# Yxxxb/LAVT-RS

Hardware: NVIDIA B200
Metric: LAVT-RS fwd clips/s (8x384^2) (higher is better)
Workload: dtype bf16

## Files before the change

### include/lavt_b200.h

```cpp
#ifndef LAVT_B200_H_
#define LAVT_B200_H_

#include <stdint.h>

#ifdef __cplusplus
extern "C" {
#endif

#define LAVT_ABI_VERSION 3

#define LAVT_ERR_SHAPE 1
#define LAVT_ERR_CUDA 2
#define LAVT_ERR_ARCH 3

enum { LAVT_ACT_NONE = 0, LAVT_ACT_GELU = 1, LAVT_ACT_RELU = 2, LAVT_ACT_TANH = 3, LAVT_ACT_SIGMOID = 4 };

typedef struct lavt_win_geom {
  int32_t B, D, H, W;
  int32_t wd, wh, ww;
  int32_t sd, sh, sw;
  int32_t nwd, nwh, nww;
  int32_t N;
  int32_t Wd, Wh, Ww;
} lavt_win_geom_t;
// ... 20 lines not shown
int lavt_abi_version(void);
int lavt_check_device(void);

int lavt_gemm_bf16(const void* A, int64_t lda, const void* Wt, int64_t ldw, int32_t M, int32_t N, int32_t K,
                   const lavt_epilogue_t* epi, void* stream);

int lavt_conv3x3_bf16(const void* x_nhwc, int64_t ldx, int32_t n_img, int32_t H, int32_t W, int32_t Cin,
                      const void* Wt, int32_t Cout, const lavt_epilogue_t* epi, void* stream);

int lavt_conv3d_bf16(const void* x_ndhwc, int64_t ldx, int32_t n_clip, int32_t D, int32_t H, int32_t W, int32_t Cin,
                     const void* Wt, int32_t Cout, const lavt_epilogue_t* epi, void* stream);


int lavt_layernorm_rows(const float* x, int64_t ldx, int64_t M, int32_t C, const float* gamma, const float* beta,
                        float eps, void* out_bf16, float* out_f32, void* stream);

int lavt_layernorm_window_gather(const float* x, int32_t C, const lavt_win_geom_t* geom, const float* gamma,
                                 const float* beta, float eps, void* out_bf16, void* stream);

int lavt_patch_merge_layernorm(const float* x, int32_t B, int32_t D, int32_t H, int32_t W, int32_t C,
                               const float* gamma, const float* beta, float eps, void* out_bf16, void* stream);

int lavt_patch_embed_im2col(const float* x, int64_t stride_b, int64_t stride_c, int64_t stride_t, int32_t B, int32_t T,
                            int32_t H, int32_t W, void* out_bf16, void* stream);

int lavt_window_attention(const void* qkv, const float* table_t, int32_t L, int32_t nH, const lavt_win_geom_t* geom,
                          void* out_bf16, void* stream);
int lavt_window_attention_lse(const void* qkv, const float* table_t, int32_t L, int32_t nH, const lavt_win_geom_t* geom, void* out_bf16,
                              float* lse, void* stream);
int lavt_window_attention_has_lse(const lavt_win_geom_t* geom, int32_t L, int32_t nH);
// ... 160 lines not shown
```

### lavt_rs_b200/_cabi.py

```python
from __future__ import annotations

import ctypes as C
import os
from typing import Optional

import torch

_PKG = os.path.dirname(os.path.abspath(__file__))
LIB_PATH = os.environ.get("LAVT_LIB_PATH") or os.path.join(_PKG, "_lib", "liblavt_b200.so")

ACT_NONE, ACT_GELU, ACT_RELU, ACT_TANH, ACT_SIGMOID = 0, 1, 2, 3, 4


class WinGeom(C.Structure):
    _fields_ = [(n, C.c_int32) for n in
                ("B", "D", "H", "W", "wd", "wh", "ww", "sd", "sh", "sw",
                 "nwd", "nwh", "nww", "N", "Wd", "Wh", "Ww")]

    def rows(self) -> int:
        return self.B * self.nwd * self.nwh * self.nww * self.N

    def tokens(self) -> int:
        return self.B * self.D * self.H * self.W

# ... 36 lines not shown


ABI_VERSION = 3

_i32, _i64, _f32, _vp = C.c_int32, C.c_int64, C.c_float, C.c_void_p
_EP = C.POINTER(Epilogue)
_WG = C.POINTER(WinGeom)

SIGNATURES = {
    "lavt_check_device": [],
    "lavt_gemm_bf16": [_vp, _i64, _vp, _i64, _i32, _i32, _i32, _EP, _vp],
    "lavt_gemm_bf16_smallm": [_vp, _i64, _vp, _i64, _i32, _i32, _i32, _EP, _vp, _i64, _vp],
    "lavt_conv3x3_bf16": [_vp, _i64, _i32, _i32, _i32, _i32, _vp, _i32, _EP, _vp],
    "lavt_conv3d_bf16": [_vp, _i64, _i32, _i32, _i32, _i32, _i32, _vp, _i32, _EP, _vp],
    "lavt_layernorm_rows": [_vp, _i64, _i64, _i32, _vp, _vp, _f32, _vp, _vp, _vp],
    "lavt_layernorm_window_gather": [_vp, _i32, _WG, _vp, _vp, _f32, _vp, _vp],
    "lavt_patch_merge_layernorm": [_vp, _i32, _i32, _i32, _i32, _i32, _vp, _vp, _f32, _vp, _vp],
    "lavt_patch_embed_im2col": [_vp, _i64, _i64, _i64, _i32, _i32, _i32, _i32, _vp, _vp],
    "lavt_window_attention": [_vp, _vp, _i32, _i32, _WG, _vp, _vp],
    "lavt_window_attention_lse": [_vp, _vp, _i32, _i32, _WG, _vp, _vp, _vp],
    "lavt_instnorm_stats": [_vp, _i32, _i64, _i32, _f32, _vp, _vp, _vp],
    "lavt_pwam_kv": [_vp, _vp, _vp, _vp, _vp, _vp, _vp, _vp, _i32, _i32, _i32, _i32, _vp],
    "lavt_lang_project": [_vp, _vp, _vp, _vp, _vp, _vp, _vp, _i32, _i32, _i32, _i32, _vp],
    "lavt_lang_project_bwd": [_vp, _vp, _vp, _vp, _vp, _vp, _vp, _vp, _vp, _vp, _vp, _vp, _i32, _i32, _i32, _i32, _vp],
    "lavt_pwam_attend": [_vp, _vp, _vp, _vp, _vp, _vp, _i32, _i64, _i32, _i32, _i32, _vp],
    "lavt_pwam_mul_norm": [_vp, _vp, _vp, _vp, _i32, _i64, _i32, _vp],
    "lavt_instnorm_sum2": [_vp, _vp, _vp, _vp, _vp, _i32, _i64, _i32, _vp],
    "lavt_bert_embed": [_vp, _vp, _vp, _vp, _vp, _i32, _i32, _i32, _i32, _vp],
    "lavt_bert_attention": [_vp, _vp, _vp, _i32, _i32, _i32, _i32, _vp],
    "lavt_rows_to_channels_first": [_vp, _vp, _i32, _i32, _i32, _vp],
# ... 44 lines not shown
    "lavt_efn_norm_upsample": [_vp, _vp, _vp, _vp, _i32, _i64, _i32, _i32, _i32, _vp],
    "lavt_bcam_softmax_rows": [_vp, _i64, _vp, _i64, _vp, _i64, _i64, _i32, _vp],
    "lavt_bcam_transpose_pad": [_vp, _i64, _vp, _i64, _i32, _i64, _i32, _vp],
    "lavt_gemm_f32_ref": [_vp, _i64, _vp, _i64, _i32, _i32, _i32, _EP, _vp],
    "lavt_window_attention_f32_ref": [_vp, _vp, _i32, _i32, _WG, _vp, _vp],
    "lavt_layernorm_window_gather_f32": [_vp, _i32, _WG, _vp, _vp, _f32, _vp, _vp],
    "lavt_rows_affine_act": [_vp, _i32, _i64, _vp, _i64, _vp, _i64, _vp, _vp, _i32, _vp, _vp, _i64, _i64, _i32, _vp],
    "lavt_avgpool2_nhwc": [_vp, _i64, _vp, _i64, _i32, _i32, _i32, _i32, _vp],
    "lavt_append_coords": [_vp, _i64, _vp, _i32, _i32, _i32, _i32, _vp],
    "lavt_rows_add_table": [_vp, _i32, _i64, _vp, _i64, _vp, _vp, _i64, _i64, _i32, _vp],
    "lavt_mha_small": [_vp, _i64, _vp, _i64, _vp, _i64, _vp, _vp, _i64, _i32, _i32, _i32, _i32, _vp],
    "lavt_gate_transpose": [_vp, _i64, _vp, _i64, _vp, _i32, _i32, _i32, _vp],
}
EXPORTS = ["lavt_last_error", "lavt_abi_version", "lavt_instnorm_workspace_floats", "lavt_set_attention_impl", "lavt_set_attention_bwd_impl",
           "lavt_gemm_splitk_workspace_floats", "lavt_conv3x3_wgrad_workspace_floats", "lavt_gacd_workspace_floats", "lavt_conv3d_wgrad_workspace_floats", "lavt_adamw_chunk_elems", "lavt_window_attention_has_lse",
           *SIGNATURES.keys()]


def _declare(l: C.CDLL) -> None:
    l.lavt_abi_version.restype = C.c_int
    l.lavt_instnorm_workspace_floats.argtypes = [_i32, _i64, _i32]
    l.lavt_instnorm_workspace_floats.restype = C.c_int64
    l.lavt_gemm_splitk_workspace_floats.argtypes = [_i32, _i32, _i32]
    l.lavt_gemm_splitk_workspace_floats.restype = C.c_int64
    l.lavt_window_attention_has_lse.argtypes = [_WG, _i32, _i32]
    l.lavt_window_attention_has_lse.restype = C.c_int
    l.lavt_conv3x3_wgrad_workspace_floats.argtypes = [_i32, _i32, _i32, _i32, _i32]
    l.lavt_conv3x3_wgrad_workspace_floats.restype = C.c_int64
    l.lavt_conv3d_wgrad_workspace_floats.argtypes = [_i32, _i32, _i32, _i32, _i32, _i32]
    l.lavt_conv3d_wgrad_workspace_floats.restype = C.c_int64
    l.lavt_gacd_workspace_floats.argtypes = [_i32, _i64, _i32]
    l.lavt_gacd_workspace_floats.restype = C.c_int64
    l.lavt_adamw_chunk_elems.argtypes = []
    l.lavt_adamw_chunk_elems.restype = C.c_int
    l.lavt_set_attention_impl.argtypes = [_i32]
    l.lavt_set_attention_impl.restype = C.c_int
    l.lavt_set_attention_bwd_impl.argtypes = [_i32]
    l.lavt_set_attention_bwd_impl.restype = C.c_int
    for name, argtypes in SIGNATURES.items():
        fn = getattr(l, name)
        fn.argtypes = argtypes
# ... 179 lines not shown
        raise LavtError(f"{name} must be contiguous")
    return t


def layernorm_rows(x: torch.Tensor, gamma, beta, *, out_bf16=None, out_f32=None, eps: float = 1e-5) -> None:
    _req(x, torch.float32, "x")
    M, Cn = x.shape
    for t, dt, nm in ((out_bf16, torch.bfloat16, "out_bf16"), (out_f32, torch.float32, "out_f32")):
        if t is not None:
            _c(t, dt, nm)
    check(lib().lavt_layernorm_rows(x.data_ptr(), x.stride(0), M, Cn, _c(gamma, torch.float32, "gamma").data_ptr(),
                                    _c(beta, torch.float32, "beta").data_ptr(), eps, ptr(out_bf16), ptr(out_f32),
                                    stream_ptr()), "lavt_layernorm_rows")


def layernorm_window_gather(x: torch.Tensor, geom: WinGeom, gamma, beta, out_bf16: torch.Tensor, eps: float = 1e-5) -> None:
    _c(x, torch.float32, "x")
    Cn = x.shape[-1]
    if x.numel() != geom.tokens() * Cn or out_bf16.numel() != geom.rows() * Cn:
        raise LavtError("window gather: tensor sizes do not match the geometry")
    check(lib().lavt_layernorm_window_gather(x.data_ptr(), Cn, C.byref(geom), _c(gamma, torch.float32, "gamma").data_ptr(),
                                             _c(beta, torch.float32, "beta").data_ptr(), eps,
                                             _c(out_bf16, torch.bfloat16, "out").data_ptr(), stream_ptr()),
          "lavt_layernorm_window_gather")


def patch_merge_layernorm(x: torch.Tensor, B, D, H, W, gamma, beta, out_bf16: torch.Tensor, eps: float = 1e-5) -> None:
    _c(x, torch.float32, "x")
    Cn = x.shape[-1]
    check(lib().lavt_patch_merge_layernorm(x.data_ptr(), B, D, H, W, Cn, _c(gamma, torch.float32, "gamma").data_ptr(),
# ... 699 lines not shown
```

### lavt_rs_b200/csrc/cabi.cu

```cuda
#include "../../include/lavt_b200.h"
#include "common.cuh"
#include "gemm_tc.cuh"
#include "kernels.cuh"

#include <cstring>

namespace lavt {
const char* last_error();
int gemm_dispatch(const void* A, long long lda, const void* Bw, long long ldb, const GemmParams& p,
                  cudaStream_t stream);

static_assert(sizeof(lavt_win_geom_t) == sizeof(WinGeom), "public/private window geometry mismatch");

static int fill_epilogue(GemmParams& p, const lavt_epilogue_t* e) {
  LAVT_REQUIRE(e != nullptr, "epilogue pointer is NULL");
  p.cscale = e->cscale;
  p.bias = e->bias;
  p.act = e->act;
  p.mul = static_cast<const __nv_bfloat16*>(e->mul);
  p.ldm = e->ldm;
  p.mul_act = e->mul_act;
  p.out_pre = static_cast<__nv_bfloat16*>(e->out_pre);
  p.pre_mode = e->pre_mode;
  LAVT_REQUIRE(e->pre_mode == 0 || (e->pre_mode == 1 && e->out_pre && e->act == LAVT_ACT_GELU),
// ... 95 lines not shown
}

static inline cudaStream_t S(void* s) { return static_cast<cudaStream_t>(s); }
static inline const __nv_bfloat16* CB(const void* p) { return static_cast<const __nv_bfloat16*>(p); }
static inline __nv_bfloat16* MB(void* p) { return static_cast<__nv_bfloat16*>(p); }

int lavt_layernorm_rows(const float* x, int64_t ldx, int64_t M, int32_t C, const float* gamma, const float* beta,
                        float eps, void* out_bf16, float* out_f32, void* stream) {
  LnParams p;
  std::memset(&p, 0, sizeof(p));
  p.x = x; p.ldx = ldx; p.gamma = gamma; p.beta = beta; p.out_bf16 = MB(out_bf16); p.out_f32 = out_f32;
  p.M = M; p.C = C; p.eps = eps;
  return ln_rows_dispatch(MODE_IDENTITY, p, S(stream));
}

int lavt_layernorm_window_gather(const float* x, int32_t C, const lavt_win_geom_t* geom, const float* gamma,
                                 const float* beta, float eps, void* out_bf16, void* stream) {
  LAVT_REQUIRE(geom != nullptr, "window gather: geometry is NULL");
  LnParams p;
  std::memset(&p, 0, sizeof(p));
  std::memcpy(&p.win, geom, sizeof(WinGeom));
  p.x = x; p.ldx = C; p.gamma = gamma; p.beta = beta; p.out_bf16 = MB(out_bf16);
  p.M = 1LL * geom->B * geom->nwd * geom->nwh * geom->nww * geom->N; p.C = C; p.eps = eps;
  return ln_rows_dispatch(MODE_WINDOW, p, S(stream));
}

int lavt_patch_merge_layernorm(const float* x, int32_t B, int32_t D, int32_t H, int32_t W, int32_t C,
                               const float* gamma, const float* beta, float eps, void* out_bf16, void* stream) {
  LnParams p;
  std::memset(&p, 0, sizeof(p));
// ... 424 lines not shown
```

### lavt_rs_b200/csrc/common.cuh

```cuda
#pragma once

#include <cuda.h>
#include <cuda_bf16.h>
#include <cuda_runtime.h>
#include <stdint.h>
#include <string.h>

#define LAVT_OK 0
#define LAVT_ERR_SHAPE 1
#define LAVT_ERR_CUDA 2
#define LAVT_ERR_ARCH 3

namespace lavt {

void set_last_error(const char* fmt, ...);
int check_cuda(cudaError_t e, const char* what);
#define LAVT_CUDA(call)                                   \
  do {                                                    \
    int _rc = ::lavt::check_cuda((call), #call);          \
    if (_rc != LAVT_OK) return _rc;                       \
  } while (0)
#define LAVT_LAUNCH_CHECK(name)                           \
  do {                                                    \
    int _rc = ::lavt::check_cuda(cudaGetLastError(), name); \
// ... 75 lines not shown
}

__device__ __forceinline__ uint32_t pack_bf16x2(float lo, float hi) {
  __nv_bfloat162 v = __floats2bfloat162_rn(lo, hi);
  return *reinterpret_cast<uint32_t*>(&v);
}
__device__ __forceinline__ float2 unpack_bf16x2(uint32_t u) {
  __nv_bfloat162 v = *reinterpret_cast<__nv_bfloat162*>(&u);
  return __bfloat1622float2(v);
}

__device__ __forceinline__ float gelu_erf(float x) {
  return 0.5f * x * (1.0f + erff(x * 0.70710678118654752440f));
}

__device__ __forceinline__ void mbar_init(uint64_t* bar, uint32_t count) {
  asm volatile("mbarrier.init.shared::cta.b64 [%0], %1;" ::"r"(smem_u32(bar)), "r"(count));
}
__device__ __forceinline__ void fence_mbar_init() {
  asm volatile("fence.mbarrier_init.release.cluster;" ::: "memory");
}
__device__ __forceinline__ void mbar_expect_tx(uint64_t* bar, uint32_t bytes) {
  asm volatile("mbarrier.arrive.expect_tx.shared::cta.b64 _, [%0], %1;" ::"r"(smem_u32(bar)),
               "r"(bytes)
               : "memory");
}
__device__ __forceinline__ void mbar_arrive(uint64_t* bar) {
  asm volatile("mbarrier.arrive.shared::cta.b64 _, [%0];" ::"r"(smem_u32(bar)) : "memory");
}
__device__ __forceinline__ bool mbar_try_wait(uint64_t* bar, uint32_t parity) {
// ... 250 lines not shown
```

### lavt_rs_b200/csrc/gemm_tc.cu

```cuda
#include "common.cuh"
#include "gemm_tc.cuh"

#include <cstdio>
#include <cstdlib>
#include <cstring>

namespace lavt {

constexpr int GEMM_BM = 128;
constexpr int GEMM_BK = 64;

template <int GEMM_BN, int GEMM_STAGES, int EPI_WGS, int CTA2 = 0>
struct GemmSmem {
  static constexpr int A_BYTES = GEMM_BM * GEMM_BK * 2;
  static constexpr int B_BYTES = (CTA2 ? GEMM_BN / 2 : GEMM_BN) * GEMM_BK * 2;
  static constexpr int STAGE_BYTES = A_BYTES + B_BYTES;
  static constexpr int RING_BYTES = GEMM_STAGES * STAGE_BYTES;
  static constexpr int BAR_OFF = RING_BYTES;
  static constexpr int VEC_OFF = BAR_OFF + 256;
  static constexpr int VEC_TILE_BYTES = EPI_WGS * 2 * GEMM_BN * 4;
  static constexpr int TOTAL = VEC_OFF + VEC_TILE_BYTES + 1024 ;
  static constexpr int THREADS = 128 + 128 * EPI_WGS;
  static constexpr int MIN_CTAS = (EPI_WGS == 1) ? 2 : 1;
  static constexpr int ACC = (MIN_CTAS == 2) ? 2 : 512 / GEMM_BN;
};

__device__ __forceinline__ float ex2_approx(float x) {
  float y;
  asm("ex2.approx.ftz.f32 %0, %1;" : "=f"(y) : "f"(x));
  return y;
}
__device__ __forceinline__ float rcp_approx(float x) {
  float y;
  asm("rcp.approx.ftz.f32 %0, %1;" : "=f"(y) : "f"(x));
  return y;
}
__device__ __forceinline__ uint64_t pk2(float lo, float hi) {
  uint64_t r;
  asm("mov.b64 %0, {%1, %2};" : "=l"(r) : "f"(lo), "f"(hi));
  return r;
}
__device__ __forceinline__ void upk2(uint64_t v, float& lo, float& hi) { asm("mov.b64 {%0, %1}, %2;" : "=f"(lo), "=f"(hi) : "l"(v)); }
__device__ __forceinline__ uint64_t fma2(uint64_t a, uint64_t b, uint64_t c) {
  uint64_t r;
  asm("fma.rn.f32x2 %0, %1, %2, %3;" : "=l"(r) : "l"(a), "l"(b), "l"(c));
  return r;
}
__device__ __forceinline__ uint64_t mul2(uint64_t a, uint64_t b) {
  uint64_t r;
  asm("mul.rn.f32x2 %0, %1, %2;" : "=l"(r) : "l"(a), "l"(b));
  return r;
}
__device__ __forceinline__ void gelu_erf2(float& x0, float& x1) {
  const uint64_t x = pk2(x0, x1);
  float z0, z1;
  upk2(mul2(x, pk2(0.70710678118654752f, 0.70710678118654752f)), z0, z1);
  z0 = fminf(fmaxf(z0, -3.0f), 3.0f);
  z1 = fminf(fmaxf(z1, -3.0f), 3.0f);
  const uint64_t z = pk2(z0, z1);
  const uint64_t t = mul2(z, z);
  constexpr float K = 1.0000220904f;
  uint64_t p = pk2(4.0742095563e-08f * K, 4.0742095563e-08f * K);
  p = fma2(p, t, pk2(-1.9448222676e-06f * K, -1.9448222676e-06f * K));
  p = fma2(p, t, pk2(4.1060515983e-05f * K, 4.1060515983e-05f * K));
  p = fma2(p, t, pk2(-5.1103678896e-04f * K, -5.1103678896e-04f * K));
  p = fma2(p, t, pk2(4.2354270142e-03f * K, 4.2354270142e-03f * K));
  p = fma2(p, t, pk2(-2.5102860078e-02f * K, -2.5102860078e-02f * K));
  p = fma2(p, t, pk2(1.1107933337e-01f * K, 1.1107933337e-01f * K));
  p = fma2(p, t, pk2(-3.7531487405e-01f * K, -3.7531487405e-01f * K));
  p = fma2(p, t, pk2(1.1282684285e+00f * K, 1.1282684285e+00f * K));
  const uint64_t e = mul2(z, p);
  const uint64_t hx = mul2(x, pk2(0.5f, 0.5f));
  upk2(fma2(hx, e, hx), x0, x1);
}
__device__ __forceinline__ void gelu_both2(float& x0, float& x1, float& d0, float& d1) {
  const uint64_t x = pk2(x0, x1);
  float z0, z1;
  upk2(mul2(x, pk2(0.70710678118654752f, 0.70710678118654752f)), z0, z1);
  const uint64_t zz = pk2(z0, z1);
  float q0, q1;
  upk2(mul2(zz, zz), q0, q1);
  const float e0 = ex2_approx(-1.4426950408889634f * q0), e1 = ex2_approx(-1.4426950408889634f * q1);
  z0 = fminf(fmaxf(z0, -3.0f), 3.0f);
  z1 = fminf(fmaxf(z1, -3.0f), 3.0f);
  const uint64_t z = pk2(z0, z1);
  const uint64_t t = mul2(z, z);
  constexpr float K = 1.0000220904f;
  uint64_t p = pk2(4.0742095563e-08f * K, 4.0742095563e-08f * K);
// ... 4 lines not shown
  p = fma2(p, t, pk2(-2.5102860078e-02f * K, -2.5102860078e-02f * K));
  p = fma2(p, t, pk2(1.1107933337e-01f * K, 1.1107933337e-01f * K));
  p = fma2(p, t, pk2(-3.7531487405e-01f * K, -3.7531487405e-01f * K));
  p = fma2(p, t, pk2(1.1282684285e+00f * K, 1.1282684285e+00f * K));
  const uint64_t Phi = fma2(mul2(z, p), pk2(0.5f, 0.5f), pk2(0.5f, 0.5f));
  const uint64_t xs = mul2(x, pk2(0.3989422804014327f, 0.3989422804014327f));
  upk2(fma2(xs, pk2(e0, e1), Phi), d0, d1);
  upk2(mul2(x, Phi), x0, x1);
}
__device__ __forceinline__ void gelu_grad2(float& x0, float& x1) {
  float d0, d1;
  gelu_both2(x0, x1, d0, d1);
  x0 = d0;
  x1 = d1;
}
__device__ __forceinline__ void ldg_v8(uint32_t* r, const void* p) {
  asm volatile("ld.global.v8.b32 {%0, %1, %2, %3, %4, %5, %6, %7}, [%8];"
               : "=r"(r[0]), "=r"(r[1]), "=r"(r[2]), "=r"(r[3]), "=r"(r[4]), "=r"(r[5]), "=r"(r[6]), "=r"(r[7])
               : "l"(p));
}
__device__ __forceinline__ void stg_v8(void* p, const uint32_t* r) {
  asm volatile("st.global.v8.b32 [%0], {%1, %2, %3, %4, %5, %6, %7, %8};" ::"l"(p), "r"(r[0]), "r"(r[1]), "r"(r[2]),
               "r"(r[3]), "r"(r[4]), "r"(r[5]), "r"(r[6]), "r"(r[7])
               : "memory");
}
__device__ __forceinline__ float tanh_fast(float x) {
  const float e = ex2_approx(x * 2.8853900817779268f);
  return fmaf(-2.0f, rcp_approx(e + 1.0f), 1.0f);
}

template <int GEMM_BN, int GEMM_STAGES, int EPI_WGS, int CTA2 = 0, int SIMPLE = 0>
__global__ void __launch_bounds__(GemmSmem<GEMM_BN, GEMM_STAGES, EPI_WGS, CTA2>::THREADS, GemmSmem<GEMM_BN, GEMM_STAGES, EPI_WGS, CTA2>::MIN_CTAS)
gemm_bf16_tc_kernel(const __grid_constant__ CUtensorMap tmA, const __grid_constant__ CUtensorMap tmB,
                    const GemmParams p, const int m_tiles, const int vec_all, long long* const trace_buf) {
  using L = GemmSmem<GEMM_BN, GEMM_STAGES, EPI_WGS, CTA2>;
  const int crank = CTA2 ? static_cast<int>(cluster_ctarank()) : 0;
  const int wid0 = CTA2 ? static_cast<int>(blockIdx.x >> 1) : static_cast<int>(blockIdx.x);
  const int wstep = CTA2 ? static_cast<int>(gridDim.x >> 1) : static_cast<int>(gridDim.x);
  extern __shared__ uint8_t smem_raw[];
  uint8_t* smem = smem_raw + ((1024u - (smem_u32(smem_raw) & 1023u)) & 1023u);
// ... 576 lines not shown
```

### lavt_rs_b200/csrc/kernels.cuh

```cuda
#pragma once
#include "common.cuh"
#include "geom.cuh"

namespace lavt {

enum { MODE_IDENTITY = 0, MODE_WINDOW = 1, MODE_MERGE = 2 };

struct LnParams {
  const float* x;
  long long ldx;
  const float* gamma;
  const float* beta;
  __nv_bfloat16* out_bf16;
  float* out_f32;
  long long M;
  int C;
  float eps;
  WinGeom win;
  int mB, mD, mH, mW;
};
int ln_rows_dispatch(int mode, const LnParams& p, cudaStream_t st);
int im2col_patch4_dispatch(const float* x, long long sB, long long sC, long long sT, __nv_bfloat16* out, int B, int T, int H,
                           int W, cudaStream_t st);
long long colstats_workspace_floats(int B, long long n, int C);
int colstats_dispatch(const float* x, float* stats, float* workspace, int B, long long n, int C, float eps, cudaStream_t st);
int instnorm_sum2_dispatch(const float* a, const float* sa, const float* b, const float* sb, float* out, int B, long long n,
                           int C, cudaStream_t st);
int pwam_mul_dispatch(const __nv_bfloat16* vis, const float* lang, const float* stats, __nv_bfloat16* out, int B,
                      long long n, int C, cudaStream_t st);

struct AttnParams {
  const __nv_bfloat16* qkv;
  const float* table_t;
  __nv_bfloat16* out;
  int C, nH, L;
  WinGeom win;
  float* lse;
};
int window_attn_dispatch(const AttnParams& p, cudaStream_t st);
int attn_impl_setting(int set);
enum class AttnKernel { TC3, TC2, MMA };
AttnKernel window_attn_choose(const AttnParams& p);
bool window_attn_tc2_supported(const AttnParams& p);
int window_attn_tc2_dispatch(const AttnParams& p, cudaStream_t st);
// ... 104 lines not shown
```

### lavt_rs_b200/engine.py

```python
from __future__ import annotations

from typing import Dict, Optional, Sequence, Tuple

import torch

from . import _cabi as K
from .geometry import window_geometry

LAUNCHES = 0
PRECISION = "bf16"


def set_precision(mode: str) -> str:
    global PRECISION
    if mode not in ("bf16", "fp32"):
        raise ValueError("precision must be 'bf16' or 'fp32'")
    prev, PRECISION = PRECISION, mode
    return prev


def _count(n: int = 1) -> None:
    global LAUNCHES
    LAUNCHES += n

# ... 81 lines not shown
        return s, b
    qkv_s, qkv_b = pw.get("qkv_sb", [blk.attn.qkv.weight] + ([blk.attn.qkv.bias] if blk.attn.qkv.bias is not None else []), _qscale)
    proj_w = pw.get("proj_w", [blk.attn.proj.weight], lambda: _bf16(blk.attn.proj.weight))
    fc1_w = pw.get("fc1_w", [blk.mlp.fc1.weight], lambda: _bf16(blk.mlp.fc1.weight))
    fc2_w = pw.get("fc2_w", [blk.mlp.fc2.weight], lambda: _bf16(blk.mlp.fc2.weight))
    table_t = pw.get("table_t", [blk.attn.relative_position_bias_table],
                     lambda: _f32(blk.attn.relative_position_bias_table.t()))

    xw = ws.get("xw", (rows, C), torch.bfloat16, dev)
    K.layernorm_window_gather(x, geom, blk.norm1.weight, blk.norm1.bias, xw, eps=blk.norm1.eps)
    qkv = ws.get("qkv", (rows, 3 * C), torch.bfloat16, dev)
    K.gemm_bf16(xw, qkv_w, cscale=qkv_s, bias=qkv_b, out_bf16=qkv)
    att = ws.get("att", (rows, C), torch.bfloat16, dev)
    K.window_attention(qkv, table_t, geom, att)
    K.gemm_bf16(att, proj_w, bias=blk.attn.proj.bias.detach(), resid=x, out_f32=x, win=geom)
    h1 = ws.get("ln2", (n, C), torch.bfloat16, dev)
    K.layernorm_rows(x, blk.norm2.weight, blk.norm2.bias, out_bf16=h1, eps=blk.norm2.eps)
    hid = ws.get("hid", (n, fc1_w.shape[0]), torch.bfloat16, dev)
    K.gemm_bf16(h1, fc1_w, bias=blk.mlp.fc1.bias.detach(), act=K.ACT_GELU, out_bf16=hid)
    K.gemm_bf16(hid, fc2_w, bias=blk.mlp.fc2.bias.detach(), resid=x, out_f32=x, out_bf16=xb_out)
    _count(7)


def _swin_block_fp32(x: torch.Tensor, blk, geom, ws: Workspace, xb_out: Optional[torch.Tensor]) -> None:
    n, C = x.shape
    dev = x.device
    rows, nH = geom.rows(), blk.num_heads
    hd = C // nH
    s = torch.ones(3 * C, device=dev, dtype=torch.float32)
    s[:C] = hd ** -0.5 * 1.4426950408889634
# ... 684 lines not shown
```

Before: 281.7.

## Fuse Swin MLP (LayerNorm, fc1+GELU, fc2+residual) into one persistent tcgen05 kernel

Adds a persistent warp-specialized kernel that runs LayerNorm2, fc1 with GELU, and fc2 with bias and residual for Swin blocks with C in {128,256}. The hidden activation stays in tensor memory and shared memory instead of making a round trip through global memory. The kernel uses a TMA weight ring, double-buffered A tiles and TMEM accumulators, and the engine calls it in place of three launches. It adds a complex mbarrier pipeline, which brings deadlock risk, and it only covers the two smaller channel widths.

After: 287.2, median of 6. +1.9%, better.

```diff
diff --git a/include/lavt_b200.h b/include/lavt_b200.h
--- a/include/lavt_b200.h
+++ b/include/lavt_b200.h
@@ -58,6 +58,10 @@
 
 int lavt_layernorm_rows(const float* x, int64_t ldx, int64_t M, int32_t C, const float* gamma, const float* beta,
                         float eps, void* out_bf16, float* out_f32, void* stream);
+
+int lavt_swin_mlp_supported(int32_t C, int32_t hidden);
+int lavt_swin_mlp_bf16(float* x, int64_t M, int32_t C, int32_t hidden, const float* gamma, const float* beta, float eps, const void* w1,
+                       const float* b1, const void* w2, const float* b2, void* xb_out, void* stream);
 
 int lavt_layernorm_window_gather(const float* x, int32_t C, const lavt_win_geom_t* geom, const float* gamma,
                                  const float* beta, float eps, void* out_bf16, void* stream);
diff --git a/lavt_rs_b200/_cabi.py b/lavt_rs_b200/_cabi.py
--- a/lavt_rs_b200/_cabi.py
+++ b/lavt_rs_b200/_cabi.py
@@ -74,6 +74,7 @@
     "lavt_conv3x3_bf16": [_vp, _i64, _i32, _i32, _i32, _i32, _vp, _i32, _EP, _vp],
     "lavt_conv3d_bf16": [_vp, _i64, _i32, _i32, _i32, _i32, _i32, _vp, _i32, _EP, _vp],
     "lavt_layernorm_rows": [_vp, _i64, _i64, _i32, _vp, _vp, _f32, _vp, _vp, _vp],
+    "lavt_swin_mlp_bf16": [_vp, _i64, _i32, _i32, _vp, _vp, _f32, _vp, _vp, _vp, _vp, _vp, _vp],
     "lavt_layernorm_window_gather": [_vp, _i32, _WG, _vp, _vp, _f32, _vp, _vp],
     "lavt_patch_merge_layernorm": [_vp, _i32, _i32, _i32, _i32, _i32, _vp, _vp, _f32, _vp, _vp],
     "lavt_patch_embed_im2col": [_vp, _i64, _i64, _i64, _i32, _i32, _i32, _i32, _vp, _vp],
@@ -148,7 +149,7 @@
 }
 EXPORTS = ["lavt_last_error", "lavt_abi_version", "lavt_instnorm_workspace_floats", "lavt_set_attention_impl", "lavt_set_attention_bwd_impl",
            "lavt_gemm_splitk_workspace_floats", "lavt_conv3x3_wgrad_workspace_floats", "lavt_gacd_workspace_floats", "lavt_conv3d_wgrad_workspace_floats", "lavt_adamw_chunk_elems", "lavt_window_attention_has_lse",
-           *SIGNATURES.keys()]
+           "lavt_swin_mlp_supported", *SIGNATURES.keys()]
 
 
 def _declare(l: C.CDLL) -> None:
@@ -159,6 +160,8 @@
     l.lavt_gemm_splitk_workspace_floats.restype = C.c_int64
     l.lavt_window_attention_has_lse.argtypes = [_WG, _i32, _i32]
     l.lavt_window_attention_has_lse.restype = C.c_int
+    l.lavt_swin_mlp_supported.argtypes = [_i32, _i32]
+    l.lavt_swin_mlp_supported.restype = C.c_int
     l.lavt_conv3x3_wgrad_workspace_floats.argtypes = [_i32, _i32, _i32, _i32, _i32]
     l.lavt_conv3x3_wgrad_workspace_floats.restype = C.c_int64
     l.lavt_conv3d_wgrad_workspace_floats.argtypes = [_i32, _i32, _i32, _i32, _i32, _i32]
@@ -368,6 +371,30 @@
                                     stream_ptr()), "lavt_layernorm_rows")
 
 
+def swin_mlp_supported(C: int, hidden: int) -> bool:
+    return bool(lib().lavt_swin_mlp_supported(int(C), int(hidden)))
+
+
+def swin_mlp(x: torch.Tensor, gamma, beta, w1: torch.Tensor, b1, w2: torch.Tensor, b2, *, xb_out=None, eps: float = 1e-5) -> None:
+    _c(x, torch.float32, "x")
+    M, Cn = x.shape
+    _c(w1, torch.bfloat16, "w1")
+    _c(w2, torch.bfloat16, "w2")
+    hidden = w1.shape[0]
+    if tuple(w1.shape) != (hidden, Cn) or tuple(w2.shape) != (Cn, hidden):
+        raise LavtError(f"swin mlp: weight shapes {tuple(w1.shape)} / {tuple(w2.shape)} do not match C={Cn}")
+    if xb_out is not None and tuple(xb_out.shape) != (M, Cn):
+        raise LavtError("swin mlp: xb_out must have the shape of x")
+    t0 = TIMER.begin()
+    check(lib().lavt_swin_mlp_bf16(x.data_ptr(), M, Cn, hidden, _c(gamma, torch.float32, "gamma").data_ptr(),
+                                   _c(beta, torch.float32, "beta").data_ptr(), eps, w1.data_ptr(), _c(b1, torch.float32, "b1").data_ptr(),
+                                   w2.data_ptr(), _c(b2, torch.float32, "b2").data_ptr(),
+                                   ptr(_c(xb_out, torch.bfloat16, "xb_out") if xb_out is not None else None), stream_ptr()),
+          "lavt_swin_mlp_bf16")
+    TIMER.end(t0, "swin_mlp_tc_kernel", 4.0 * M * Cn * hidden, 8.0 * M * Cn + 4.0 * Cn * hidden + (2.0 * M * Cn if xb_out is not None else 0.0),
+              f"M{M} C{Cn} hidden{hidden}")
+
+
 def layernorm_window_gather(x: torch.Tensor, geom: WinGeom, gamma, beta, out_bf16: torch.Tensor, eps: float = 1e-5) -> None:
     _c(x, torch.float32, "x")
     Cn = x.shape[-1]
diff --git a/lavt_rs_b200/csrc/cabi.cu b/lavt_rs_b200/csrc/cabi.cu
--- a/lavt_rs_b200/csrc/cabi.cu
+++ b/lavt_rs_b200/csrc/cabi.cu
@@ -133,6 +133,18 @@
   return ln_rows_dispatch(MODE_IDENTITY, p, S(stream));
 }
 
+int lavt_swin_mlp_supported(int32_t C, int32_t hidden) { return swin_mlp_supported(C, hidden) ? 1 : 0; }
+
+int lavt_swin_mlp_bf16(float* x, int64_t M, int32_t C, int32_t hidden, const float* gamma, const float* beta, float eps, const void* w1,
+                       const float* b1, const void* w2, const float* b2, void* xb_out, void* stream) {
+  SwinMlpParams p;
+  std::memset(&p, 0, sizeof(p));
+  p.x = x; p.xb_out = MB(xb_out); p.gamma = gamma; p.beta = beta; p.eps = eps;
+  p.w1 = CB(w1); p.b1 = b1; p.w2 = CB(w2); p.b2 = b2;
+  p.M = M; p.C = C; p.hidden = hidden;
+  return swin_mlp_dispatch(p, S(stream));
+}
+
 int lavt_layernorm_window_gather(const float* x, int32_t C, const lavt_win_geom_t* geom, const float* gamma,
                                  const float* beta, float eps, void* out_bf16, void* stream) {
   LAVT_REQUIRE(geom != nullptr, "window gather: geometry is NULL");
diff --git a/lavt_rs_b200/csrc/common.cuh b/lavt_rs_b200/csrc/common.cuh
--- a/lavt_rs_b200/csrc/common.cuh
+++ b/lavt_rs_b200/csrc/common.cuh
@@ -113,6 +113,55 @@
   return 0.5f * x * (1.0f + erff(x * 0.70710678118654752440f));
 }
 
+__device__ __forceinline__ uint64_t pk2(float lo, float hi) {
+  uint64_t r;
+  asm("mov.b64 %0, {%1, %2};" : "=l"(r) : "f"(lo), "f"(hi));
+  return r;
+}
+__device__ __forceinline__ void upk2(uint64_t v, float& lo, float& hi) { asm("mov.b64 {%0, %1}, %2;" : "=f"(lo), "=f"(hi) : "l"(v)); }
+__device__ __forceinline__ uint64_t fma2(uint64_t a, uint64_t b, uint64_t c) {
+  uint64_t r;
+  asm("fma.rn.f32x2 %0, %1, %2, %3;" : "=l"(r) : "l"(a), "l"(b), "l"(c));
+  return r;
+}
+__device__ __forceinline__ uint64_t mul2(uint64_t a, uint64_t b) {
+  uint64_t r;
+  asm("mul.rn.f32x2 %0, %1, %2;" : "=l"(r) : "l"(a), "l"(b));
+  return r;
+}
+__device__ __forceinline__ void gelu_erf2(float& x0, float& x1) {
+  const uint64_t x = pk2(x0, x1);
+  float z0, z1;
+  upk2(mul2(x, pk2(0.70710678118654752f, 0.70710678118654752f)), z0, z1);
+  z0 = fminf(fmaxf(z0, -3.0f), 3.0f);
+  z1 = fminf(fmaxf(z1, -3.0f), 3.0f);
+  const uint64_t z = pk2(z0, z1);
+  const uint64_t t = mul2(z, z);
+  constexpr float K = 1.0000220904f;
+  uint64_t p = pk2(4.0742095563e-08f * K, 4.0742095563e-08f * K);
+  p = fma2(p, t, pk2(-1.9448222676e-06f * K, -1.9448222676e-06f * K));
+  p = fma2(p, t, pk2(4.1060515983e-05f * K, 4.1060515983e-05f * K));
+  p = fma2(p, t, pk2(-5.1103678896e-04f * K, -5.1103678896e-04f * K));
+  p = fma2(p, t, pk2(4.2354270142e-03f * K, 4.2354270142e-03f * K));
+  p = fma2(p, t, pk2(-2.5102860078e-02f * K, -2.5102860078e-02f * K));
+  p = fma2(p, t, pk2(1.1107933337e-01f * K, 1.1107933337e-01f * K));
+  p = fma2(p, t, pk2(-3.7531487405e-01f * K, -3.7531487405e-01f * K));
+  p = fma2(p, t, pk2(1.1282684285e+00f * K, 1.1282684285e+00f * K));
+  const uint64_t e = mul2(z, p);
+  const uint64_t hx = mul2(x, pk2(0.5f, 0.5f));
+  upk2(fma2(hx, e, hx), x0, x1);
+}
+__device__ __forceinline__ void ldg_v8(uint32_t* r, const void* p) {
+  asm volatile("ld.global.v8.b32 {%0, %1, %2, %3, %4, %5, %6, %7}, [%8];"
+               : "=r"(r[0]), "=r"(r[1]), "=r"(r[2]), "=r"(r[3]), "=r"(r[4]), "=r"(r[5]), "=r"(r[6]), "=r"(r[7])
+               : "l"(p));
+}
+__device__ __forceinline__ void stg_v8(void* p, const uint32_t* r) {
+  asm volatile("st.global.v8.b32 [%0], {%1, %2, %3, %4, %5, %6, %7, %8};" ::"l"(p), "r"(r[0]), "r"(r[1]), "r"(r[2]),
+               "r"(r[3]), "r"(r[4]), "r"(r[5]), "r"(r[6]), "r"(r[7])
+               : "memory");
+}
+
 __device__ __forceinline__ void mbar_init(uint64_t* bar, uint32_t count) {
   asm volatile("mbarrier.init.shared::cta.b64 [%0], %1;" ::"r"(smem_u32(bar)), "r"(count));
 }
diff --git a/lavt_rs_b200/csrc/gemm_tc.cu b/lavt_rs_b200/csrc/gemm_tc.cu
--- a/lavt_rs_b200/csrc/gemm_tc.cu
+++ b/lavt_rs_b200/csrc/gemm_tc.cu
@@ -34,44 +34,6 @@
   float y;
   asm("rcp.approx.ftz.f32 %0, %1;" : "=f"(y) : "f"(x));
   return y;
-}
-__device__ __forceinline__ uint64_t pk2(float lo, float hi) {
-  uint64_t r;
-  asm("mov.b64 %0, {%1, %2};" : "=l"(r) : "f"(lo), "f"(hi));
-  return r;
-}
-__device__ __forceinline__ void upk2(uint64_t v, float& lo, float& hi) { asm("mov.b64 {%0, %1}, %2;" : "=f"(lo), "=f"(hi) : "l"(v)); }
-__device__ __forceinline__ uint64_t fma2(uint64_t a, uint64_t b, uint64_t c) {
-  uint64_t r;
-  asm("fma.rn.f32x2 %0, %1, %2, %3;" : "=l"(r) : "l"(a), "l"(b), "l"(c));
-  return r;
-}
-__device__ __forceinline__ uint64_t mul2(uint64_t a, uint64_t b) {
-  uint64_t r;
-  asm("mul.rn.f32x2 %0, %1, %2;" : "=l"(r) : "l"(a), "l"(b));
-  return r;
-}
-__device__ __forceinline__ void gelu_erf2(float& x0, float& x1) {
-  const uint64_t x = pk2(x0, x1);
-  float z0, z1;
-  upk2(mul2(x, pk2(0.70710678118654752f, 0.70710678118654752f)), z0, z1);
-  z0 = fminf(fmaxf(z0, -3.0f), 3.0f);
-  z1 = fminf(fmaxf(z1, -3.0f), 3.0f);
-  const uint64_t z = pk2(z0, z1);
-  const uint64_t t = mul2(z, z);
-  constexpr float K = 1.0000220904f;
-  uint64_t p = pk2(4.0742095563e-08f * K, 4.0742095563e-08f * K);
-  p = fma2(p, t, pk2(-1.9448222676e-06f * K, -1.9448222676e-06f * K));
-  p = fma2(p, t, pk2(4.1060515983e-05f * K, 4.1060515983e-05f * K));
-  p = fma2(p, t, pk2(-5.1103678896e-04f * K, -5.1103678896e-04f * K));
-  p = fma2(p, t, pk2(4.2354270142e-03f * K, 4.2354270142e-03f * K));
-  p = fma2(p, t, pk2(-2.5102860078e-02f * K, -2.5102860078e-02f * K));
-  p = fma2(p, t, pk2(1.1107933337e-01f * K, 1.1107933337e-01f * K));
-  p = fma2(p, t, pk2(-3.7531487405e-01f * K, -3.7531487405e-01f * K));
-  p = fma2(p, t, pk2(1.1282684285e+00f * K, 1.1282684285e+00f * K));
-  const uint64_t e = mul2(z, p);
-  const uint64_t hx = mul2(x, pk2(0.5f, 0.5f));
-  upk2(fma2(hx, e, hx), x0, x1);
 }
 __device__ __forceinline__ void gelu_both2(float& x0, float& x1, float& d0, float& d1) {
   const uint64_t x = pk2(x0, x1);
@@ -106,16 +68,6 @@
   x0 = d0;
   x1 = d1;
 }
-__device__ __forceinline__ void ldg_v8(uint32_t* r, const void* p) {
-  asm volatile("ld.global.v8.b32 {%0, %1, %2, %3, %4, %5, %6, %7}, [%8];"
-               : "=r"(r[0]), "=r"(r[1]), "=r"(r[2]), "=r"(r[3]), "=r"(r[4]), "=r"(r[5]), "=r"(r[6]), "=r"(r[7])
-               : "l"(p));
-}
-__device__ __forceinline__ void stg_v8(void* p, const uint32_t* r) {
-  asm volatile("st.global.v8.b32 [%0], {%1, %2, %3, %4, %5, %6, %7, %8};" ::"l"(p), "r"(r[0]), "r"(r[1]), "r"(r[2]),
-               "r"(r[3]), "r"(r[4]), "r"(r[5]), "r"(r[6]), "r"(r[7])
-               : "memory");
-}
 __device__ __forceinline__ float tanh_fast(float x) {
   const float e = ex2_approx(x * 2.8853900817779268f);
   return fmaf(-2.0f, rcp_approx(e + 1.0f), 1.0f);
diff --git a/lavt_rs_b200/csrc/kernels.cuh b/lavt_rs_b200/csrc/kernels.cuh
--- a/lavt_rs_b200/csrc/kernels.cuh
+++ b/lavt_rs_b200/csrc/kernels.cuh
@@ -28,6 +28,22 @@
                            int C, cudaStream_t st);
 int pwam_mul_dispatch(const __nv_bfloat16* vis, const float* lang, const float* stats, __nv_bfloat16* out, int B,
                       long long n, int C, cudaStream_t st);
+
+struct SwinMlpParams {
+  float* x;
+  __nv_bfloat16* xb_out;
+  const float* gamma;
+  const float* beta;
+  float eps;
+  const __nv_bfloat16* w1;
+  const float* b1;
+  const __nv_bfloat16* w2;
+  const float* b2;
+  long long M;
+  int C, hidden;
+};
+bool swin_mlp_supported(int C, int hidden);
+int swin_mlp_dispatch(const SwinMlpParams& p, cudaStream_t st);
 
 struct AttnParams {
   const __nv_bfloat16* qkv;
diff --git a/lavt_rs_b200/csrc/swin_mlp_tc.cu b/lavt_rs_b200/csrc/swin_mlp_tc.cu
--- /dev/null
+++ b/lavt_rs_b200/csrc/swin_mlp_tc.cu
@@ -0,0 +1,427 @@
+#include "common.cuh"
+#include "attn_tc_ptx.cuh"
+#include "kernels.cuh"
+
+#include <cstdio>
+
+namespace lavt {
+
+namespace {
+
+constexpr int MLP_BM = 128;
+constexpr int MLP_CH = 128;
+constexpr int MLP_STAGE_BYTES = 32 * 1024;
+constexpr int MLP_THREADS = 640;
+
+template <int C>
+struct MlpCfg {
+  static constexpr int HID = 4 * C;
+  static constexpr int NCH = HID / MLP_CH;
+  static constexpr int SPC = C / 128;
+  static constexpr int STAGES = (C == 128) ? 4 : 3;
+  static constexpr int A_BYTES = MLP_BM * C * 2;
+  static constexpr int NACC = (512 - 2 * MLP_CH) / C;
+  static constexpr int RING_OFF = 2 * A_BYTES;
+  static constexpr int BAR_OFF = RING_OFF + STAGES * MLP_STAGE_BYTES;
+  static constexpr int SMEM = BAR_OFF + 256 + 1024;
+  static constexpr int LPR = C / 16;
+  static constexpr int RPS = 32 / LPR;
+};
+
+__device__ __forceinline__ uint32_t sw128_offset(int r, int k) {
+  const int atom = k >> 6, byte = (k & 63) * 2;
+  return atom * (MLP_BM * 128) + r * 128 + ((((byte >> 4) ^ (r & 7))) << 4) + (byte & 15);
+}
+
+#ifdef LAVT_MLP_WATCHDOG
+__device__ int* mlp_abort_flag() {
+  __shared__ int flag;
+  return &flag;
+}
+__device__ __forceinline__ void mlp_wait(uint64_t* bar, uint32_t parity, int line) {
+  const long long t0 = clock64();
+  while (!mbar_try_wait(bar, parity)) {
+    const bool aborted = *reinterpret_cast<volatile int*>(mlp_abort_flag()) != 0;
+    if (aborted || clock64() - t0 > 2000000000LL) {
+      if ((threadIdx.x & 31) == 0)
+        printf("[swin_mlp stuck] block %d warp %d line %d parity %u%s\n", blockIdx.x, threadIdx.x >> 5, line, parity, aborted ? " (snapshot)" : "");
+      *reinterpret_cast<volatile int*>(mlp_abort_flag()) = 1;
+      return;
+    }
+  }
+}
+#else
+__device__ __forceinline__ void mlp_wait(uint64_t* bar, uint32_t parity, int) { mbar_wait(bar, parity); }
+#endif
+#define MLP_WAIT(bar, parity) mlp_wait((bar), (parity), __LINE__)
+
+}
+
+template <int C>
+__global__ void __launch_bounds__(MLP_THREADS, 1)
+swin_mlp_tc_kernel(const __grid_constant__ CUtensorMap tmW1, const __grid_constant__ CUtensorMap tmW2, float* __restrict__ x,
+                   __nv_bfloat16* __restrict__ xb_out, const float* __restrict__ gamma, const float* __restrict__ beta, float eps,
+                   const float* __restrict__ b1, const float* __restrict__ b2, const int M) {
+  using L = MlpCfg<C>;
+  extern __shared__ uint8_t smem_raw[];
+  uint8_t* smem = smem_raw + ((1024u - (smem_u32(smem_raw) & 1023u)) & 1023u);
+  uint64_t* full_bar = reinterpret_cast<uint64_t*>(smem + L::BAR_OFF);
+  uint64_t* empty_bar = full_bar + L::STAGES;
+  uint64_t* a_full = empty_bar + L::STAGES;
+  uint64_t* a_empty = a_full + 2;
+  uint64_t* hid_full = a_empty + 2;
+  uint64_t* hidb_full = hid_full + 2;
+  uint64_t* hid_empty = hidb_full + 2;
+  uint64_t* acc_full = hid_empty + 2;
+  uint64_t* acc_empty = acc_full + 2;
+  uint32_t* tmem_ptr_smem = reinterpret_cast<uint32_t*>(acc_empty + 2);
+
+  const int warp = threadIdx.x >> 5;
+  const int lane = threadIdx.x & 31;
+  const int n_tiles = (M + MLP_BM - 1) / MLP_BM;
+
+  if (warp == 0 && lane == 0) {
+    tma_prefetch_desc(&tmW1);
+    tma_prefetch_desc(&tmW2);
+  }
+  if (warp == 1 && lane == 0) {
+    for (int s = 0; s < L::STAGES; ++s) {
+      mbar_init(&full_bar[s], 1);
+      mbar_init(&empty_bar[s], 1);
+    }
+    for (int i = 0; i < 2; ++i) {
+      mbar_init(&a_full[i], 4);
+      mbar_init(&a_empty[i], 1);
+      mbar_init(&hid_full[i], 1);
+      mbar_init(&hidb_full[i], 4);
+      mbar_init(&hid_empty[i], 1);
+      mbar_init(&acc_full[i], 1);
+      mbar_init(&acc_empty[i], 4);
+    }
+    fence_mbar_init();
+  }
+#ifdef LAVT_MLP_WATCHDOG
+  if (threadIdx.x == 0) *mlp_abort_flag() = 0;
+#endif
+  if (warp == 2) tmem_alloc(tmem_ptr_smem, 512);
+  pdl_wait();
+  pdl_launch_dependents();
+  tc_fence_before();
+  __syncthreads();
+  tc_fence_after();
+  const uint32_t tmem_base = *tmem_ptr_smem;
+  const uint32_t tmem_acc = tmem_base + 2 * MLP_CH;
+
+  if (warp == 0) {
+    if (lane == 0) {
+      int it = 0;
+      auto slot = [&](int s) -> uint8_t* {
+        MLP_WAIT(&empty_bar[s], ((it / L::STAGES) & 1) ^ 1);
+        mbar_expect_tx(&full_bar[s], MLP_STAGE_BYTES);
+        return smem + L::RING_OFF + s * MLP_STAGE_BYTES;
+      };
+      for (int tile = blockIdx.x; tile < n_tiles; tile += gridDim.x) {
+        for (int j = 0; j <= L::NCH; ++j) {
+          if (j < L::NCH) {
+            for (int q = 0; q < L::SPC; ++q, ++it) {
+              const int s = it % L::STAGES;
+              uint8_t* dst = slot(s);
+              tma_load_2d(dst, &tmW1, &full_bar[s], (2 * q) * 64, j * MLP_CH);
+              tma_load_2d(dst + 16384, &tmW1, &full_bar[s], (2 * q + 1) * 64, j * MLP_CH);
+            }
+          }
+          if (j >= 1) {
+            const int jj = j - 1;
+            for (int q = 0; q < L::SPC; ++q, ++it) {
+              const int s = it % L::STAGES;
+              uint8_t* dst = slot(s);
+              if (C == 128) {
+                tma_load_2d(dst, &tmW2, &full_bar[s], jj * MLP_CH, 0);
+                tma_load_2d(dst + 16384, &tmW2, &full_bar[s], jj * MLP_CH + 64, 0);
+              } else {
+                tma_load_2d(dst, &tmW2, &full_bar[s], jj * MLP_CH + q * 64, 0);
+              }
+            }
+          }
+        }
+      }
+    }
+  } else if (warp == 1) {
+    if (lane == 0) {
+      constexpr uint32_t idesc1 = make_idesc_bf16_f32(MLP_BM, MLP_CH);
+      constexpr uint32_t idesc2 = make_idesc_bf16_f32(MLP_BM, C);
+      int it = 0, lt = 0;
+      for (int tile = blockIdx.x; tile < n_tiles; tile += gridDim.x, ++lt) {
+        const int ab = lt & 1;
+        const uint32_t tacc = tmem_acc + (lt % L::NACC) * C;
+        const int prev = lt - L::NACC;
+        MLP_WAIT(&a_full[ab], (lt >> 1) & 1);
+        tc_fence_after();
+        const uint32_t sa = smem_u32(smem + ab * L::A_BYTES);
+        for (int j = 0; j <= L::NCH; ++j) {
+          if (j < L::NCH) {
+            const int b = j & 1;
+            const uint32_t u = static_cast<uint32_t>((lt * L::NCH + j) >> 1);
+            MLP_WAIT(&hid_empty[b], (u & 1) ^ 1);
+            tc_fence_after();
+            const uint32_t td = tmem_base + b * MLP_CH;
+            for (int q = 0; q < L::SPC; ++q, ++it) {
+              const int s = it % L::STAGES;
+              MLP_WAIT(&full_bar[s], (it / L::STAGES) & 1);
+              tc_fence_after();
+              const uint32_t sb = smem_u32(smem + L::RING_OFF + s * MLP_STAGE_BYTES);
+#pragma unroll
+              for (int h = 0; h < 2; ++h) {
+                const int atom = 2 * q + h;
+                const uint64_t da = make_kmajor_sw128_desc(sa + atom * (MLP_BM * 128));
+                const uint64_t db = make_kmajor_sw128_desc(sb + h * 16384);
+#pragma unroll
+                for (int k = 0; k < 4; ++k) umma_bf16_ss(td, da + 2 * k, db + 2 * k, idesc1, (atom | k) != 0);
+              }
+              umma_commit(&empty_bar[s]);
+            }
+            umma_commit(&hid_full[b]);
+            if (j == L::NCH - 1) umma_commit(&a_empty[ab]);
+          }
+          if (j >= 1) {
+            const int jj = j - 1, b = jj & 1;
+            const uint32_t u = static_cast<uint32_t>((lt * L::NCH + jj) >> 1);
+            MLP_WAIT(&hidb_full[b], u & 1);
+            if (jj == 0 && prev >= 0) MLP_WAIT(&acc_empty[prev & 1], (prev >> 1) & 1);
+            tc_fence_after();
+            const uint32_t ta = tmem_base + b * MLP_CH;
+            for (int q = 0; q < L::SPC; ++q, ++it) {
+              const int s = it % L::STAGES;
+              MLP_WAIT(&full_bar[s], (it / L::STAGES) & 1);
+              tc_fence_after();
+              const uint32_t sb = smem_u32(smem + L::RING_OFF + s * MLP_STAGE_BYTES);
+#pragma unroll
+              for (int h = 0; h < 2 / L::SPC; ++h) {
+                const int hh = q * (2 / L::SPC) + h;
+                const uint64_t db = make_kmajor_sw128_desc(sb + h * 16384);
+#pragma unroll
+                for (int k = 0; k < 4; ++k)
+                  umma_bf16_ts(tacc, ta + hh * 32 + 8 * k, db + 2 * k, idesc2, (jj | hh | k) != 0);
+              }
+              umma_commit(&empty_bar[s]);
+            }
+            umma_commit(&hid_empty[b]);
+            if (jj == L::NCH - 1) umma_commit(&acc_full[ab]);
+          }
+        }
+      }
+    }
+  } else if (warp >= 4 && warp < 12) {
+    const int g = (warp - 4) >> 2;
+    const int ew = warp & 3;
+    const uint32_t tb = tmem_base + g * MLP_CH + (static_cast<uint32_t>(ew * 32) << 16);
+    int lt = 0;
+    for (int tile = blockIdx.x; tile < n_tiles; tile += gridDim.x, ++lt) {
+      for (int j = g; j < L::NCH; j += 2) {
+        const uint32_t u = static_cast<uint32_t>((lt * L::NCH + j) >> 1);
+        MLP_WAIT(&hid_full[g], u & 1);
+        tc_fence_after();
+        const float4* bi4 = reinterpret_cast<const float4*>(b1 + j * MLP_CH);
+#pragma unroll 1
+        for (int c = 0; c < MLP_CH / 32; ++c) {
+          uint32_t v[32];
+          tmem_ld_32x32b_x32(tb + c * 32, v);
+          tmem_ld_wait();
+          float f[32];
+#pragma unroll
+          for (int q = 0; q < 8; ++q) {
+            const float4 bi = __ldg(bi4 + c * 8 + q);
+            f[4 * q] = __uint_as_float(v[4 * q]) + bi.x;
+            f[4 * q + 1] = __uint_as_float(v[4 * q + 1]) + bi.y;
+            f[4 * q + 2] = __uint_as_float(v[4 * q + 2]) + bi.z;
+            f[4 * q + 3] = __uint_as_float(v[4 * q + 3]) + bi.w;
+          }
+          uint32_t pk[16];
+#pragma unroll
+          for (int e = 0; e < 16; ++e) {
+            gelu_erf2(f[2 * e], f[2 * e + 1]);
+            pk[e] = pack_bf16x2(f[2 * e], f[2 * e + 1]);
+          }
+          tmem_st_x16(tb + c * 16, pk);
+        }
+        tmem_st_wait();
+        tc_fence_before();
+        __syncwarp();
+        if (lane == 0) mbar_arrive(&hidb_full[g]);
+      }
+    }
+  } else if (warp >= 12) {
+    const int r = (warp - 12) >> 2;
+    const int ew = warp & 3;
+    uint8_t* const sa = smem + r * L::A_BYTES;
+    constexpr int LPR = L::LPR, RPS = L::RPS;
+    const int sl = lane % LPR, sr = lane / LPR;
+    constexpr float inv_cn = 1.0f / static_cast<float>(C);
+    auto prefetch_rows = [&](int tile) {
+      const int row = tile * MLP_BM + ew * 32;
+      if (lane == 0 && tile < n_tiles && row < M) {
+        const int nrows = min(32, M - row);
+        asm volatile("cp.async.bulk.prefetch.L2.global [%0], %1;" ::"l"(x + static_cast<size_t>(row) * C), "r"(nrows * C * 4) : "memory");
+      }
+    };
+    prefetch_rows(blockIdx.x + r * gridDim.x);
+    int lt = r;
+    for (int tile = blockIdx.x + r * gridDim.x; tile < n_tiles; tile += 2 * gridDim.x, lt += 2) {
+      const int row0 = tile * MLP_BM;
+      prefetch_rows(tile + 2 * gridDim.x);
+      MLP_WAIT(&a_empty[r], ((lt >> 1) & 1) ^ 1);
+      auto load_rows = [&](int rb, float4 (&v)[4]) {
+        const int m = row0 + ew * 32 + rb + sr;
+        const float4* src = reinterpret_cast<const float4*>(x + static_cast<size_t>(m < M ? m : 0) * C);
+#pragma unroll
+        for (int i = 0; i < 4; ++i) v[i] = m < M ? __ldg(src + i * LPR + sl) : make_float4(0.f, 0.f, 0.f, 0.f);
+      };
+#pragma unroll 1
+      for (int rb = 0; rb < 32; rb += RPS) {
+        float4 v[4];
+        load_rows(rb, v);
+        const bool live = row0 + ew * 32 + rb + sr < M;
+        float s = 0.f;
+#pragma unroll
+        for (int i = 0; i < 4; ++i) s += (v[i].x + v[i].y) + (v[i].z + v[i].w);
+#pragma unroll
+        for (int o = LPR / 2; o > 0; o >>= 1) s += __shfl_xor_sync(0xffffffffu, s, o);
+        const float mean = s * inv_cn;
+        float ss = 0.f;
+#pragma unroll
+        for (int i = 0; i < 4; ++i) {
+          const float a = v[i].x - mean, b = v[i].y - mean, c = v[i].z - mean, d = v[i].w - mean;
+          ss += (a * a + b * b) + (c * c + d * d);
+        }
+#pragma unroll
+        for (int o = LPR / 2; o > 0; o >>= 1) ss += __shfl_xor_sync(0xffffffffu, ss, o);
+        const float rstd = rsqrtf(ss * inv_cn + eps);
+        const int tr = ew * 32 + rb + sr;
+#pragma unroll
+        for (int i = 0; i < 4; ++i) {
+          float4 y = make_float4(0.f, 0.f, 0.f, 0.f);
+          if (live) {
+            const float4 gm = __ldg(reinterpret_cast<const float4*>(gamma) + i * LPR + sl);
+            const float4 bt = __ldg(reinterpret_cast<const float4*>(beta) + i * LPR + sl);
+            y.x = (v[i].x - mean) * rstd * gm.x + bt.x;
+            y.y = (v[i].y - mean) * rstd * gm.y + bt.y;
+            y.z = (v[i].z - mean) * rstd * gm.z + bt.z;
+            y.w = (v[i].w - mean) * rstd * gm.w + bt.w;
+          }
+          *reinterpret_cast<uint2*>(sa + sw128_offset(tr, 4 * (i * LPR + sl))) = make_uint2(pack_bf16x2(y.x, y.y), pack_bf16x2(y.z, y.w));
+        }
+      }
+      fence_proxy_async_smem();
+      __syncwarp();
+      if (lane == 0) mbar_arrive(&a_full[r]);
+
+      const int m = row0 + ew * 32 + lane;
+      const bool live = m < M;
+      float* xrow = x + static_cast<size_t>(live ? m : 0) * C;
+      __nv_bfloat16* brow = (xb_out && live) ? xb_out + static_cast<size_t>(m) * C : nullptr;
+      const uint32_t ta = tmem_acc + (lt % L::NACC) * C + (static_cast<uint32_t>(ew * 32) << 16);
+      MLP_WAIT(&acc_full[r], (lt >> 1) & 1);
+      tc_fence_after();
+      uint32_t rr[16], rn[16];
+      if (live) {
+        ldg_v8(&rr[0], xrow);
+        ldg_v8(&rr[8], xrow + 8);
+      }
+#pragma unroll 1
+      for (int c = 0; c < C / 16; ++c) {
+        if (live && c + 1 < C / 16) {
+          ldg_v8(&rn[0], xrow + (c + 1) * 16);
+          ldg_v8(&rn[8], xrow + (c + 1) * 16 + 8);
+        }
+        uint32_t v[16];
+        tmem_ld_32x32b_x16(ta + c * 16, v);
+        tmem_ld_wait();
+        if (c == C / 16 - 1) {
+          tc_fence_before();
+          __syncwarp();
+          if (lane == 0) mbar_arrive(&acc_empty[r]);
+        }
+        if (!live) continue;
+        const float4* bi4 = reinterpret_cast<const float4*>(b2 + c * 16);
+#pragma unroll
+        for (int q = 0; q < 4; ++q) {
+          const float4 bi = __ldg(bi4 + q);
+          rr[4 * q] = __float_as_uint((__uint_as_float(v[4 * q]) + bi.x) + __uint_as_float(rr[4 * q]));
+          rr[4 * q + 1] = __float_as_uint((__uint_as_float(v[4 * q + 1]) + bi.y) + __uint_as_float(rr[4 * q + 1]));
+          rr[4 * q + 2] = __float_as_uint((__uint_as_float(v[4 * q + 2]) + bi.z) + __uint_as_float(rr[4 * q + 2]));
+          rr[4 * q + 3] = __float_as_uint((__uint_as_float(v[4 * q + 3]) + bi.w) + __uint_as_float(rr[4 * q + 3]));
+        }
+        stg_v8(xrow + c * 16, &rr[0]);
+        stg_v8(xrow + c * 16 + 8, &rr[8]);
+        if (brow) {
+#pragma unroll
+          for (int e = 0; e < 8; ++e) v[e] = pack_bf16x2(__uint_as_float(rr[2 * e]), __uint_as_float(rr[2 * e + 1]));
+          stg_v8(brow + c * 16, v);
+        }
+#pragma unroll
+        for (int e = 0; e < 16; ++e) rr[e] = rn[e];
+      }
+    }
+  }
+
+  tc_fence_before();
+  __syncthreads();
+  if (warp == 2) {
+    tc_fence_after();
+    tmem_dealloc(tmem_base, 512);
+  }
+}
+
+bool swin_mlp_supported(int C, int hidden) { return (C == 128 || C == 256) && hidden == 4 * C; }
+
+template <int C>
+static int launch_swin_mlp(const SwinMlpParams& p, cudaStream_t st) {
+  using L = MlpCfg<C>;
+  CUtensorMap tmW1, tmW2;
+  {
+    uint64_t dims[2] = {(uint64_t)C, (uint64_t)L::HID};
+    uint64_t strides[1] = {(uint64_t)C * 2};
+    uint32_t box[2] = {64, 128};
+    int rc = make_tmap_bf16(&tmW1, p.w1, 2, dims, strides, box, CU_TENSOR_MAP_SWIZZLE_128B);
+    if (rc) return rc;
+  }
+  {
+    uint64_t dims[2] = {(uint64_t)L::HID, (uint64_t)C};
+    uint64_t strides[1] = {(uint64_t)L::HID * 2};
+    uint32_t box[2] = {64, (uint32_t)C};
+    int rc = make_tmap_bf16(&tmW2, p.w2, 2, dims, strides, box, CU_TENSOR_MAP_SWIZZLE_128B);
+    if (rc) return rc;
+  }
+  auto kfn = swin_mlp_tc_kernel<C>;
+  static bool configured = false;
+  if (!configured) {
+    LAVT_CUDA(cudaFuncSetAttribute(kfn, cudaFuncAttributeMaxDynamicSharedMemorySize, L::SMEM));
+    configured = true;
+  }
+  static int sms = 0;
+  if (sms == 0) {
+    int dev = 0;
+    if (cudaGetDevice(&dev) != cudaSuccess || cudaDeviceGetAttribute(&sms, cudaDevAttrMultiProcessorCount, dev) != cudaSuccess || sms <= 0)
+      sms = 148;
+  }
+  const long long tiles = (p.M + MLP_BM - 1) / MLP_BM;
+  const int grid = static_cast<int>(tiles < sms ? tiles : sms);
+  LAVT_CUDA(launch_pdl(kfn, dim3(grid), dim3(MLP_THREADS), L::SMEM, st, 1, tmW1, tmW2, p.x, p.xb_out, p.gamma, p.beta, p.eps, p.b1, p.b2,
+                       static_cast<int>(p.M)));
+  LAVT_LAUNCH_CHECK("swin_mlp_tc_kernel");
+  return LAVT_OK;
+}
+
+int swin_mlp_dispatch(const SwinMlpParams& p, cudaStream_t st) {
+  LAVT_REQUIRE(swin_mlp_supported(p.C, p.hidden), "swin mlp: C=%d hidden=%d not supported (C in {128, 256}, hidden == 4C)", p.C, p.hidden);
+  LAVT_REQUIRE(p.M > 0 && p.M < (1LL << 31) - MLP_BM, "swin mlp: M=%lld out of range", p.M);
+  LAVT_REQUIRE(p.x && p.gamma && p.beta && p.w1 && p.b1 && p.w2 && p.b2, "swin mlp: NULL operand");
+  LAVT_REQUIRE((reinterpret_cast<uintptr_t>(p.x) | reinterpret_cast<uintptr_t>(p.xb_out)) % 32 == 0 &&
+                   (reinterpret_cast<uintptr_t>(p.gamma) | reinterpret_cast<uintptr_t>(p.beta) | reinterpret_cast<uintptr_t>(p.b1) |
+                    reinterpret_cast<uintptr_t>(p.b2)) % 16 == 0,
+               "swin mlp: x / xb_out must be 32-byte and the vectors 16-byte aligned");
+  if (p.C == 128) return launch_swin_mlp<128>(p, st);
+  return launch_swin_mlp<256>(p, st);
+}
+
+}
diff --git a/lavt_rs_b200/engine.py b/lavt_rs_b200/engine.py
--- a/lavt_rs_b200/engine.py
+++ b/lavt_rs_b200/engine.py
@@ -119,6 +119,11 @@
     att = ws.get("att", (rows, C), torch.bfloat16, dev)
     K.window_attention(qkv, table_t, geom, att)
     K.gemm_bf16(att, proj_w, bias=blk.attn.proj.bias.detach(), resid=x, out_f32=x, win=geom)
+    if K.swin_mlp_supported(C, fc1_w.shape[0]):
+        K.swin_mlp(x, blk.norm2.weight, blk.norm2.bias, fc1_w, blk.mlp.fc1.bias.detach(), fc2_w, blk.mlp.fc2.bias.detach(),
+                   xb_out=xb_out, eps=blk.norm2.eps)
+        _count(5)
+        return
     h1 = ws.get("ln2", (n, C), torch.bfloat16, dev)
     K.layernorm_rows(x, blk.norm2.weight, blk.norm2.bias, out_bf16=h1, eps=blk.norm2.eps)
     hid = ws.get("hid", (n, fc1_w.shape[0]), torch.bfloat16, dev)
```
